# albertfgu/diffwave-sashimi

Hardware: AMD Instinct MI355X
Metric: audio samples/sec (generate.py-style reverse-diffusion sampling, T=200) (higher is better)
Workload: dtype f32-equivalent (3-term bf16 split, 6 products, fp32 accumulate); 1 GPU; wnet_h256_d36_T200; backbone=wavenet, batch_per_gpu=16, L=16000, T=200, parallelism=independent clips per GPU, no collective, sampler=hipGraph replay, on-device Philox noise

## Files before the change

### diffwave-sashimi_amd/csrc/bf16_split.h

```cpp
#pragma once
#include <hip/hip_runtime.h>

namespace dws {

typedef __bf16 bx_bf16x8 __attribute__((ext_vector_type(8)));
typedef __bf16 bx_bf16x4 __attribute__((ext_vector_type(4)));
typedef float bx_f32x16 __attribute__((ext_vector_type(16)));

__device__ __forceinline__ void split3(float x, __bf16& p0, __bf16& p1, __bf16& p2) {
    p0 = (__bf16)x;
    const float r1 = x - (float)p0;
    p1 = (__bf16)r1;
    const float r2 = r1 - (float)p1;
    p2 = (__bf16)r2;
}

__device__ __forceinline__ void split3x4(const float (&x)[4], bx_bf16x4& p0, bx_bf16x4& p1, bx_bf16x4& p2) {
#pragma unroll
    for (int e = 0; e < 4; ++e) {
        __bf16 a, b, c;
        split3(x[e], a, b, c);
        p0[e] = a; p1[e] = b; p2[e] = c;
    }
}
// ... 15 lines not shown
    out[1] = bx_bf16x8{a1, b1, z, z, z, z, z, z};
    out[2] = bx_bf16x8{a2, b2, z, z, z, z, z, z};
}

struct SplitBf16x3 {
    typedef bx_bf16x8 v8;
    typedef bx_bf16x4 v4;
    static constexpr int NT = 3, NP = 6;
    static constexpr bool SCALED = false;
    static constexpr float SX = 1.f, SG = 1.f;
    __device__ static constexpr int ia(int t) { return BX6_IA[t]; }
    __device__ static constexpr int ib(int t) { return BX6_IB[t]; }
    __device__ static __forceinline__ bx_f32x16 mfma(const v8& a, const v8& b, const bx_f32x16& c) {
        return __builtin_amdgcn_mfma_f32_32x32x16_bf16(a, b, c, 0, 0, 0);
    }
    __device__ static __forceinline__ void split4(const float (&x)[4], v4 (&p)[3]) { split3x4(x, p[0], p[1], p[2]); }
    __device__ static __forceinline__ void split1(float x, v8 (&out)[3], int i) {
        __bf16 a, b, c;
        split3(x, a, b, c);
        out[0][i] = a; out[1][i] = b; out[2][i] = c;
    }
    __device__ static __forceinline__ void rank2(float v0, float v1, bool lower_half, v8 (&out)[3]) { frag_rank2(v0, v1, lower_half, out); }
    __device__ static __forceinline__ void bits(float x, unsigned short (&b)[3]) {
        __bf16 p0, p1, p2;
        split3(x, p0, p1, p2);
        b[0] = __builtin_bit_cast(unsigned short, p0); b[1] = __builtin_bit_cast(unsigned short, p1); b[2] = __builtin_bit_cast(unsigned short, p2);
    }
    __device__ static __forceinline__ v8 bvals(float v0, float v1) {
        const __bf16 z = (__bf16)0.f;
        return v8{(__bf16)v0, (__bf16)v1, z, z, z, z, z, z};
    }
};

typedef _Float16 hx_f16x8 __attribute__((ext_vector_type(8)));
typedef _Float16 hx_f16x4 __attribute__((ext_vector_type(4)));
struct SplitF16x2 {
    typedef hx_f16x8 v8;
// ... 44 lines not shown
```

### diffwave-sashimi_amd/csrc/wavenet.h

```cpp
#pragma once
#include "dws_common.h"

namespace dws {

constexpr int WN_LAYER_KC = 32;
constexpr int WN_BX3_KC = 16;

struct WnLayerArgs {
    const float* x_in;
    float* x_out;
    float* skip;
    const float* part_t;
    int part_t_bstride;
    const float* A1;
    const float* A2;
    const float* Abt;
    int abt_bstride;
    const int* step_idx;
    int abt_tstride, part_t_tstride;
    const float* Wd;
    const float* Wr;
    const float* Ws;
    const float* bias1;
    const float* bias2;
// ... 36 lines not shown
bool wn_layer_mfma_supported(int C, int S);
int launch_wn_layer_mfma(int C, int S, const WnLayerArgs& a, hipStream_t s);
int launch_wn_layer_generic(int C, int S, const WnLayerArgs& a, hipStream_t s);
bool wn_final_mfma_supported(int S);
bool wn_layer_wino_supported(int C, int S);
int launch_wino_dconv(const float* w, float* out, int C, hipStream_t s);
int launch_wn_wino_bias(const float* Wd_all, const float* part_t, float* Abt, int NL, int B, int C, hipStream_t s);
int launch_wn_layer_wino(int C, int S, const WnLayerArgs& a, hipStream_t s);
bool wn_layer_bf16x3_supported(int C, int S);
int launch_wn_layer_bf16x3(int C, int S, const WnLayerArgs& a, hipStream_t s);
int launch_pack_a_bf16x3(const float* w, void* out, int M, int K, hipStream_t s);
int launch_wn_bias_tap_bf16(const float* Wd_all, const float* part_t, const float* bias1_all, void* Abt, int NL, int B, int C,
                            hipStream_t s);
enum { WN_SPLIT_BF16X6 = 0, WN_SPLIT_F16X3 = 1 };
inline int wn_split_terms(int split) { return split == WN_SPLIT_F16X3 ? 2 : 3; }
bool wn_layer_bx6_supported(int C, int S);
int launch_wn_layer_bx6(int C, int S, const WnLayerArgs& a, int split, hipStream_t s);
int launch_weight_scale(const float* w, size_t n, const float* bias, int nb, const float* bias_b, int nb_b, float* out, hipStream_t s);
int launch_pack_a1_bx6(const float* w, void* out, int C, int split, const float* scale, hipStream_t s);
int launch_pack_a_bx6(const float* w, void* out, int M, int K, int split, const float* scale, hipStream_t s);
int launch_gemm_bx6(const float* A, const float* B, float* C, int M, int N, int K, int split, float sa, float sb, hipStream_t s);
int launch_wn_final(int S, const WnFinalArgs& a, hipStream_t s);

}
```

### diffwave-sashimi_amd/csrc/wavenet_bx6.hip

```cpp
#include <cstdlib>
#include <type_traits>

#include "bf16_split.h"
#include "wavenet.h"
#include "wn_trace.h"

namespace dws {

#ifndef BX6_PF3
#define BX6_PF3 1
#endif
#ifndef BX6_PF2
#define BX6_PF2 2
#endif
#define BX6_PF(NT) ((NT) == 2 ? BX6_PF2 : BX6_PF3)
#ifndef BX6_T_SLOTS
#define BX6_T_SLOTS 0, 2, 3, 4, 6, 7, 9
#endif

typedef float bx6_f32x4 __attribute__((ext_vector_type(4)));

#ifdef BX6_ABL_NO_NT
#define BX6_NT 0
#else
// ... 120 lines not shown
    static constexpr int RAW_FLOATS = KC * 4 * NP;
    static constexpr int BOP_BYTES = (KC / 8) * 4 * NT * NP * 16;
    static constexpr int STAGE_FLOATS = 2 * RAW_FLOATS + 2 * BOP_BYTES / 4;
    static constexpr int GATE_BYTES = (C / 8) * NT * 64 * 16;
    static constexpr int MAIN_FLOATS = STAGE_FLOATS > GATE_BYTES / 4 ? STAGE_FLOATS : GATE_BYTES / 4;
    static constexpr int TR_FLOATS = 32 * 64;
    static constexpr int LDS_FLOATS = MAIN_FLOATS + WAVES * TR_FLOATS;
    static constexpr int TITEMS = (KC / 4) * NP * 2;
    static constexpr bool HALVES = WAVES == 8 && NT == 3;
    static constexpr int SW = HALVES ? WAVES / 2 : WAVES;
    static constexpr int NPIECE = KC / (2 * SW);
    static_assert(C % 32 == 0 && S % C == 0 && C % KC == 0 && KC % 16 == 0 && KC % (2 * SW) == 0 && (SW & (SW - 1)) == 0 &&
                  (!HALVES || NCB % 2 == 0) && (TITEMS % NTH == 0) && LDS_FLOATS * 4 <= 163840, "channel counts");
};

template <typename P, int C, int S, bool EXTRA>
__global__ __launch_bounds__(C * 2, (C >= 128 ? 2 : 1)) void wn_layer_bx6_kernel(WnLayerArgs a, int log2d) {
    using T = Bx6Tile<C, S, P::NT>;
    using v8 = typename P::v8;
    using v4 = typename P::v4;
    constexpr int NT = P::NT, NPR = P::NP, NA = 2 * P::NT;
    constexpr int KC = T::KC, MS = T::MS, WAVES = T::WAVES, NCB = T::NCB, NTH = T::NTH, NKB = T::NKB;
    __shared__ __attribute__((aligned(16))) float lds[T::LDS_FLOATS];
    float* const Xraw = lds;
    char* const Bop = reinterpret_cast<char*>(lds + 2 * T::RAW_FLOATS);
    char* const gt = reinterpret_cast<char*>(lds);

    const int tid = threadIdx.x;
    const int lane = tid & 63;
    const int wave = __builtin_amdgcn_readfirstlane(tid >> 6);
    const int l31 = lane & 31, lhi = lane >> 5;
    const int L = a.L, dil = 1 << log2d;
    float* const trw = lds + T::MAIN_FLOATS + wave * T::TR_FLOATS;
// ... 14 lines not shown
    const float* __restrict__ xb = a.x_in + (size_t)b * C * L;
    unsigned long long* __restrict__ trc = a.trace ? a.trace + ((size_t)blockIdx.x * WAVES + wave) * 32 : nullptr;
    auto stamp = [&](int i) {
        if (trc) {
            const unsigned long long t = __builtin_amdgcn_s_memtime();
            if (lane == 0) trc[i] = t;
        }
    };
    stamp(0);

    const int mt1[2] = {wave, C / 32 + wave};
    int mt2[1 + MS];
    mt2[0] = wave;
#pragma unroll
    for (int m = 0; m < MS; ++m) mt2[1 + m] = C / 32 + wave * MS + m;
    float av1[2][4], ab1[2], av2[1 + MS];
    {
        const float* Abt = a.Abt + (size_t)b * a.abt_bstride + step_row_off(a.step_idx, a.abt_tstride);
#pragma unroll
        for (int m = 0; m < 2; ++m) {
            const int row = mt1[m] * 32 + l31;
#pragma unroll
            for (int j = 0; j < 4; ++j) av1[m][j] = Abt[j * 2 * C + row];
            ab1[m] = a.bias1[row];
        }
#pragma unroll
        for (int m = 0; m < 1 + MS; ++m) av2[m] = a.bias2[mt2[m] * 32 + l31];
    }
    const float ws1 = P::SCALED ? a.wscale[0] : 1.f, ws2 = P::SCALED ? a.wscale[1] : 1.f;
    const float inv1 = 1.f / (ws1 * P::SX), inv2 = 1.f / (ws2 * P::SG);

    const bool al16 = (L % 4 == 0) && ((((size_t)a.x_in | (size_t)a.x_out | (size_t)a.skip) & 15) == 0);
// ... 132 lines not shown
#pragma unroll
        for (int m = 0; m < 2; ++m)
#pragma unroll
            for (int t = 0; t < NT; ++t)
#ifdef BX6_ABL_A_HOT
                dst[m][t] = __builtin_bit_cast(v8, __builtin_amdgcn_raw_buffer_load_b128(rA1, lane16, ((mt1[m] * NKB * 4) * NT + t) * 1024 + 0 * (kb + j), 0));
#else
                dst[m][t] = __builtin_bit_cast(v8, __builtin_amdgcn_raw_buffer_load_b128(rA1, lane16, (((mt1[m] * NKB + kb) * 4 + j) * NT + t) * 1024, 0));
#endif
    };

    if (stages(0)) stage_dma(0);
    if (NCB > 1 && stages(1)) stage_dma(1);
    constexpr int PF = BX6_PF(NT);
    v8 a_ring[4][2][NT];
#pragma unroll
    for (int s0 = 0; s0 < PF; ++s0) load_a1(a_ring[s0], chunk_of(0) * (KC / 16) + (s0 >> 2), s0 & 3);
    constexpr int NAF = PF * NA;
    constexpr int P16 = NPIECE + NAF, P4 = 4 * NPIECE + NAF;
    static_assert(P4 < 64, "vmcnt is a 6-bit counter");
    if (HALVES) {
        if (stages(0)) __builtin_amdgcn_s_waitcnt(0x0F70 | NAF);
    } else if (NCB > 1) {
        if (x4) __builtin_amdgcn_s_waitcnt(0x0F70 | (P16 & 15) | ((P16 >> 4) << 14));
        else __builtin_amdgcn_s_waitcnt(0x0F70 | (P4 & 15) | ((P4 >> 4) << 14));
    } else {
        __builtin_amdgcn_s_waitcnt(0x0F70 | NAF);
    }
    __syncthreads();
    stamp(1);
    {
        const float v0 = ((unsigned)(p - dil) < (unsigned)L) ? 1.f : 0.f;
        const float v1 = ((unsigned)p < (unsigned)L) ? 1.f : 0.f;
        const float v2 = ((unsigned)(p + dil) < (unsigned)L) ? 1.f : 0.f;
        const float v3 = ((unsigned)(p + 2 * dil) < (unsigned)L) ? 1.f : 0.f;
        const float bi[4] = {v0 - v2, v1 + v2, v2 - v1, v1 - v3};
        bx_f32x16 zero;
#pragma unroll
        for (int r = 0; r < 16; ++r) zero[r] = 0.f;
#pragma unroll
        for (int j = 0; j < 4; ++j) {
            const v8 bf = P::bvals(lhi ? 0.f : bi[j] * P::SX, (lhi || j != 1) ? 0.f : P::SX);
#pragma unroll
            for (int m = 0; m < 2; ++m) {
                v8 af[NT];
                P::rank2(av1[m][j] * ws1, j == 1 ? ab1[m] * ws1 : 0.f, lhi == 0, af);
// ... 60 lines not shown
        if constexpr (SPC == 4) {
            do_step(cb, std::integral_constant<int, 1>{}, std::false_type{});
            do_step(cb, std::integral_constant<int, 2>{}, std::false_type{});
            do_step(cb, std::integral_constant<int, 3>{}, std::false_type{});
        } else {
            do_step(cb, std::integral_constant<int, 1>{}, std::false_type{});
            do_step(cb, std::integral_constant<int, 2>{}, std::false_type{});
            do_step(cb, std::integral_constant<int, 3>{}, std::false_type{});
            do_step(cb, std::integral_constant<int, 4>{}, std::false_type{});
            do_step(cb, std::integral_constant<int, 5>{}, std::false_type{});
            do_step(cb, std::integral_constant<int, 6>{}, std::false_type{});
            do_step(cb, std::integral_constant<int, 7>{}, std::false_type{});
        }
    };
    static_assert((SPC == 4 || SPC == 8) && PF >= 1 && PF <= 3, "steps per chunk, prefetch distance");
    for (int cb = 0; cb < NCB; ++cb) {
#ifndef BX6_ABL_NO_STAGE
        if (cb + 2 < NCB && stages(cb + 2)) stage_dma(cb + 2);
#endif
        if (cb + 1 < NCB) do_step(cb, std::integral_constant<int, 0>{}, std::true_type{});
        else do_step(cb, std::integral_constant<int, 0>{}, std::false_type{});
        do_steps_from1(cb);
        stamp(8 + 2 * cb);
#ifndef BX6_ABL_NO_DMA_WAIT
        __builtin_amdgcn_s_waitcnt(0x0F70 | NAF);
#endif
#ifndef BX6_ABL_NO_BARRIER
        __syncthreads();
#endif
        stamp(9 + 2 * cb);
    }
    stamp(2);

    const int L4 = L * 4;
    const bool first = a.first_layer, last = a.last_layer;
    __amdgpu_buffer_rsrc_t rXo = __builtin_amdgcn_make_buffer_rsrc((void*)(a.x_out + (size_t)b * C * L), 0, C * L * 4, 0x00020000);
    __amdgpu_buffer_rsrc_t rSk = __builtin_amdgcn_make_buffer_rsrc((void*)(a.skip + (size_t)b * S * L), 0, S * L * 4, 0x00020000);
    const int p0 = ((q0 >> log2d) << (log2d + 1)) + (q0 & (dil - 1));
    int voff4;
    {
        const int n4 = (lane & 15) >> 3;
        const int pos4 = (contig ? pbase + 32 * n4 : p0 + n4 * dil) + 4 * (lane & 7);
        voff4 = (pos4 < L) ? ((lane >> 4) * L + pos4) * 4 : 0x7ffffff0;
    }
    constexpr bool PRELOAD = MS == 1;
    const int voff4s = first ? 0x7ffffff0 : voff4;
    auto load_pre = [&](int m, bx6_f32x4 (&dst)[8]) {
#pragma unroll
        for (int i = 0; i < 8; ++i) {
            if (m == 0) dst[i] = *reinterpret_cast<const bx6_f32x4*>(trw + ((lane >> 4) + 4 * i) * 64 + 4 * (lane & 15));
            else dst[i] = bx6_load_f4(rSk, voff4s, ((wave * MS + (m - 1)) * 32 + 4 * i) * L4);
        }
    };
    bx6_f32x4 pre[PRELOAD ? 1 + MS : 1][8];
    if (PRELOAD && al16) {
#pragma unroll
        for (int m = 1; m < 1 + MS; ++m) load_pre(m, pre[PRELOAD ? m : 0]);
    }

    const float* melb = (EXTRA && a.melc) ? a.melc + (size_t)(a.mel_bstride ? b : 0) * 2 * C * L : nullptr;
#pragma unroll
    for (int qd = 0; qd < 4; ++qd) {
        float g0[4], g1[4];
#pragma unroll
        for (int e = 0; e < 4; ++e) {
            const int r = qd * 4 + e;
            const int ch = wave * 32 + e + 8 * qd + 4 * lhi;
#pragma unroll
            for (int n = 0; n < 2; ++n) {
                const int pos = p + n * dil;
                float ht, hs;
                if (n == 0) {
                    ht = (acc[0][0][r] + acc[0][1][r]) + acc[0][2][r];
                    hs = (acc[1][0][r] + acc[1][1][r]) + acc[1][2][r];
                } else {
// ... 11 lines not shown
                    hb[(size_t)(C + ch) * L + pos] = hs;
                }
                const float g = bx6_gate(ht, hs) * P::SG;
                if (n == 0) g0[e] = g; else g1[e] = g;
            }
        }
        v4 s0[NT], s1[NT];
        P::split4(g0, s0);
        P::split4(g1, s1);
        char* dst = gt + ((wave * 4 + qd) * NT * 64) * 16 + lhi * 8;
#pragma unroll
        for (int t = 0; t < NT; ++t) {
            *reinterpret_cast<v4*>(dst + (t * 64 + gcol0) * 16) = s0[t];
            *reinterpret_cast<v4*>(dst + (t * 64 + gcol1) * 16) = s1[t];
        }
    }
    stamp(3);

    __amdgpu_buffer_rsrc_t rA2 = __builtin_amdgcn_make_buffer_rsrc((void*)a.A2, 0, (C + S) * C * 2 * NT, 0x00020000);
    v8 c_cur[1 + MS][NT], c_nxt[1 + MS][NT];
    auto load_a2 = [&](v8 (&dst)[1 + MS][NT], int kb, int m0) {
#pragma unroll
        for (int m = m0; m < 1 + MS; ++m)
#pragma unroll
            for (int t = 0; t < NT; ++t)
                dst[m][t] = __builtin_bit_cast(v8, __builtin_amdgcn_raw_buffer_load_b128(rA2, lane16, ((mt2[m] * NKB + kb) * NT + t) * 1024, 0));
    };
    const int rot2 = rot * (KC / 16);
    auto kblock_of = [&](int kb) { const int k = kb + rot2; return k >= NKB ? k - NKB : k; };
    bx_f32x16 acc2[1 + MS][2];
// ... 32 lines not shown
#pragma unroll
                for (int t = 0; t < NT; ++t) bq[n][t] = *reinterpret_cast<const v8*>(gk + (t * 64 + n * 32) * 16);
#pragma unroll
            for (int t = 0; t < NPR; ++t)
#pragma unroll
                for (int m = M0; m < 1 + MS; ++m)
#pragma unroll
                    for (int n = 0; n < 2; ++n)
                        acc2[m][n] = P::mfma(c_cur[m][P::ia(t)], bq[n][P::ib(t)], acc2[m][n]);
#pragma unroll
            for (int m = M0; m < 1 + MS; ++m)
#pragma unroll
                for (int t = 0; t < NT; ++t) c_cur[m][t] = c_nxt[m][t];
        }
    };
    if (last) gemm2(std::false_type{});
    else gemm2(std::true_type{});
    stamp(5);

    const float rs = 0.70710678118654752440f;
    if (al16) {
#pragma unroll
        for (int m = 0; m < 1 + MS; ++m) {
            if (m == 0 && last) continue;
            if (!PRELOAD || m == 0) load_pre(m, pre[0]);
            asm volatile("s_waitcnt lgkmcnt(0)" ::: "memory");
#pragma unroll
            for (int n = 0; n < 2; ++n)
#pragma unroll
                for (int r = 0; r < 16; ++r) trw[((r & 3) + 8 * (r >> 2) + 4 * lhi) * 64 + n * 32 + l31] = P::SCALED ? acc2[m][n][r] * inv2 : acc2[m][n][r];
            asm volatile("s_waitcnt lgkmcnt(0)" ::: "memory");
            const int row0 = (m == 0) ? wave * 32 : (wave * MS + (m - 1)) * 32;
#pragma unroll
            for (int i = 0; i < 8; ++i) {
                const bx6_f32x4 v = *reinterpret_cast<const bx6_f32x4*>(trw + ((lane >> 4) + 4 * i) * 64 + 4 * (lane & 15));
                bx6_f32x4 o = pre[PRELOAD ? m : 0][i] + v;
                if (m == 0) o = o * rs;
                bx6_store_f4(o, m == 0 ? rXo : rSk, voff4, (row0 + 4 * i) * L4);
                asm volatile("s_nop 1" ::: "memory");
            }
            asm volatile("" ::: "memory");
        }
    } else {
        int voffn[2];
#pragma unroll
        for (int n = 0; n < 2; ++n) {
            const int pos = contig ? pbase + 32 * n + l31 : p + n * dil;
            voffn[n] = (pos < L) ? (4 * lhi * L + pos) * 4 : 0x7ffffff0;
        }
#pragma unroll
        for (int n = 0; n < 2; ++n) {
            if (!last) {
                const int s0 = (wave * 32) * L4;
#pragma unroll
                for (int r = 0; r < 16; ++r) {
                    const int so = s0 + ((r & 3) + 8 * (r >> 2)) * L4;
                    const float x = __builtin_bit_cast(float, __builtin_amdgcn_raw_buffer_load_b32(rXall, voffn[n], so, 0));
// ... 9 lines not shown
                    const int so = s0 + ((r & 3) + 8 * (r >> 2)) * L4;
                    const float old = first ? 0.f : __builtin_bit_cast(float, __builtin_amdgcn_raw_buffer_load_b32(rSk, voffn[n], so, 0));
                    const float v = old + (P::SCALED ? acc2[1 + m][n][r] * inv2 : acc2[1 + m][n][r]);
                    __builtin_amdgcn_raw_buffer_store_b32(__builtin_bit_cast(unsigned, v), rSk, voffn[n], so, 0);
                }
            }
        }
    }
    stamp(6);
    if (trc) {
        __builtin_amdgcn_s_waitcnt(0);
        stamp(7);
    }
}

template <typename P, int C, int S>
static int launch_bx6_t(const WnLayerArgs& a, int log2d, hipStream_t s) {
    ProfileScope ps(P::NT == 3 ? "wn_layer_bx6" : "wn_layer_f16x3", s);
    using T = Bx6Tile<C, S, P::NT>;
    const int dil = 1 << log2d;
    const int nblk = (a.L + 2 * dil - 1) / (2 * dil);
    const int ntl = (nblk * dil + 31) / 32;
    const int ntiles = a.B * ntl;
    static const bool trace = std::getenv("DWS_BX6_TRACE") != nullptr;
    if (trace && !a.melc && !a.hsave) {
        wino_trace_launch(ntiles, T::WAVES, a, s, [&](const WnLayerArgs& at) {
            hipLaunchKernelGGL((wn_layer_bx6_kernel<P, C, S, false>), dim3(ntiles), dim3(T::NTH), 0, s, at, log2d);
        }, P::NT == 3 ? "bx6" : "f16x3");
        return DWS_OK;
    }
    if (a.melc || a.hsave) hipLaunchKernelGGL((wn_layer_bx6_kernel<P, C, S, true>), dim3(ntiles), dim3(T::NTH), 0, s, a, log2d);
    else hipLaunchKernelGGL((wn_layer_bx6_kernel<P, C, S, false>), dim3(ntiles), dim3(T::NTH), 0, s, a, log2d);
    return DWS_OK;
}

bool wn_layer_bx6_supported(int C, int S) {
    return (C == 64 && S == 64) || (C == 128 && S == 128) || (C == 128 && S == 256) || (C == 256 && S == 256);
}

template <typename P>
static int launch_bx6_p(int C, int S, const WnLayerArgs& a, int log2d, hipStream_t s) {
    if (C == 64 && S == 64) return launch_bx6_t<P, 64, 64>(a, log2d, s);
    if (C == 128 && S == 128) return launch_bx6_t<P, 128, 128>(a, log2d, s);
    if (C == 128 && S == 256) return launch_bx6_t<P, 128, 256>(a, log2d, s);
    if (C == 256 && S == 256) return launch_bx6_t<P, 256, 256>(a, log2d, s);
    return set_error(DWS_ERR_UNSUPPORTED, "wn_layer_bx6: (C=%d,S=%d) not instantiated", C, S);
}

int launch_wn_layer_bx6(int C, int S, const WnLayerArgs& a, int split, hipStream_t s) {
    int log2d = 0;
    while ((1 << log2d) < a.dilation) ++log2d;
    DWS_CHECK((1 << log2d) == a.dilation, DWS_ERR_UNSUPPORTED, "wn_layer_bx6: dilation %d is not a power of two", a.dilation);
    DWS_CHECK((int64_t)a.L + 4 * (int64_t)a.dilation < ((int64_t)1 << 28), DWS_ERR_UNSUPPORTED, "wn_layer_bx6: L too large");
    DWS_CHECK((int64_t)(C > S ? C : S) * a.L * 4 < ((int64_t)1 << 31), DWS_ERR_UNSUPPORTED,
              "wn_layer_bx6: %d channels x L=%d exceed a 2 GiB tensor per clip", C > S ? C : S, a.L);
    if (split == WN_SPLIT_F16X3) {
        DWS_CHECK(a.hsave == nullptr, DWS_ERR_UNSUPPORTED, "wn_layer_f16x3: the training forward runs with precision=f32 or bf16x6");
        DWS_CHECK(a.wscale != nullptr, DWS_ERR_INVALID, "wn_layer_f16x3: no weight scales");
        return launch_bx6_p<SplitF16x2>(C, S, a, log2d, s);
    }
    return launch_bx6_p<SplitBf16x3>(C, S, a, log2d, s);
}

template <typename P>
__global__ __launch_bounds__(64) void gemm_bx6_kernel(const float* __restrict__ A, const float* __restrict__ B, float* __restrict__ Cm,
                                                      int M, int N, int K, float sa, float sb) {
    using v8 = typename P::v8;
    const int lane = threadIdx.x, l31 = lane & 31, lhi = lane >> 5;
    const int mt = blockIdx.y, nt = blockIdx.x;
    bx_f32x16 acc;
#pragma unroll
    for (int r = 0; r < 16; ++r) acc[r] = 0.f;
    for (int kb = 0; kb < K / 16; ++kb) {
        v8 af[P::NT], bf[P::NT];
#pragma unroll
// ... 43 lines not shown
```

### diffwave-sashimi_amd/csrc/wavenet_model.hip

```cpp
#include <cmath>

#include "conditioner.h"
#include "model.h"
#include "wavenet.h"
#include "wavenet_backward.h"

namespace dws {

struct WaveNetModel : dws_model {
    int Cin, Cout, C, S, NL, cycle, Ein, Emid, Eout, MB;
    bool cond, mfma_layer, mfma_final;
    bool bf16x3 = false;
    bool bf16x6 = false;
    bool f16x3 = false;
    DevBuf wscale;
    bool wino_opt = true;
    bool wino_fits(int64_t nL) const {
        return (int64_t)std::max(C, S) * nL * 4 < ((int64_t)1 << 31) && nL + 4 * ((int64_t)1 << (cycle - 1)) < ((int64_t)1 << 28);
    }
    bool wino() const { return wino_opt && mfma_layer && !bf16x3 && !bf16x6 && !f16x3 && wn_layer_wino_supported(C, S) && (L == 0 || wino_fits(L)); }
    bool wino_rows() const { return wino() || bf16x6 || f16x3; }

    DevBuf Wi;
    std::vector<DevBuf> A1, Wrs, A2, bias2;
    DevBuf Wd_all;
    DevBuf Abt;
    DevBuf Wt_all, bt_all;
    DevBuf b1_all;
    DevBuf Wf, Af;
    DevBuf freq;
    CopyBatch stack_params, unstack_fc_t;
// ... 18 lines not shown
    DevBuf de_raw;
    bool trained_fwd = false;

    explicit WaveNetModel(const dws_model_desc& dd) {
        d = dd;
        Cin = d.in_channels; Cout = d.out_channels; C = d.res_channels; S = d.skip_channels;
        NL = d.num_res_layers; cycle = d.dilation_cycle;
        Ein = d.diffusion_step_embed_dim_in; Emid = d.diffusion_step_embed_dim_mid; Eout = d.diffusion_step_embed_dim_out;
        MB = d.mel_bands;
        cond = !d.unconditional;
        mfma_layer = wn_layer_mfma_supported(C, S);
        mfma_bwd = tapconv_mfma_supported(C, S, C, 1) && tapconv_mfma_supported(C, 2 * C, 0, 3) &&
                   tapconv_mfma_supported(S, S, 0, 1) && std::getenv("DWS_WAVENET_GENERIC_BWD") == nullptr;
        mfma_final = wn_final_mfma_supported(S);
        if (std::getenv("DWS_WN_DIRECT")) wino_opt = false;
        auto wn = [&](const std::string& p, std::vector<int64_t> vshape) {
            std::vector<int64_t> g(vshape.size(), 1);
            g[0] = vshape[0];
            add_param(p + ".bias", {vshape[0]});
            add_param(p + ".weight_g", g);
            add_param(p + ".weight_v", vshape);
        };
        wn("init_conv.0.conv", {C, Cin, 1});
        add_param("residual_layer.fc_t1.weight", {Emid, Ein});
        add_param("residual_layer.fc_t1.bias", {Emid});
        add_param("residual_layer.fc_t2.weight", {Eout, Emid});
        add_param("residual_layer.fc_t2.bias", {Eout});
        for (int n = 0; n < NL; ++n) {
            const std::string p = "residual_layer.residual_blocks." + std::to_string(n);
            add_param(p + ".fc_t.weight", {C, Eout});
// ... 34 lines not shown
                          "precision=bf16x6 is not built for (res_channels=%d, skip_channels=%d)", C, S);
                bf16x6 = true; bf16x3 = f16x3 = false; dirty = true; trained_fwd = false;
                return DWS_OK;
            }
            if (value == "f16x3") {
                DWS_CHECK(mfma_layer && wn_layer_bx6_supported(C, S), DWS_ERR_UNSUPPORTED,
                          "precision=f16x3 is not built for (res_channels=%d, skip_channels=%d)", C, S);
                f16x3 = true; bf16x3 = bf16x6 = false; dirty = true; trained_fwd = false;
                return DWS_OK;
            }
        }
        if (key == "conv_algo") {
            if (value == "winograd") { wino_opt = true; dirty = true; trained_fwd = false; return DWS_OK; }
            if (value == "direct") { wino_opt = false; dirty = true; trained_fwd = false; return DWS_OK; }
        }
        return dws_model::set_option(key, value);
    }

    float* Wd(int n) const { return Wd_all.f() + (size_t)n * 2 * C * C * 3; }

    int fold(const std::string& p, float* out, int O, int inner, hipStream_t s) {
        return launch_fold_weight_norm(P(p + ".weight_v"), P(p + ".weight_g"), out, O, inner, s);
    }

    int commit(hipStream_t s) override {
        DWS_TRY(Wi.ensure((size_t)C * Cin * 4));
        DWS_TRY(fold("init_conv.0.conv", Wi.f(), C, Cin, s));
        DWS_TRY(Wt_all.ensure((size_t)NL * C * Eout * 4));
        DWS_TRY(bt_all.ensure((size_t)NL * C * 4));
        DWS_TRY(b1_all.ensure((size_t)NL * 2 * C * 4));
        DWS_TRY(Wd_all.ensure((size_t)NL * 2 * C * C * 3 * 4));
        if (mfma_layer) DWS_TRY(tmp_pack.ensure((size_t)2 * C * 4 * C * 4));
        stack_params.begin();
        for (int n = 0; n < NL; ++n) {
            const std::string p = "residual_layer.residual_blocks." + std::to_string(n);
            stack_params.add(P(p + ".fc_t.weight"), Wt_all.f() + (size_t)n * C * Eout, (size_t)C * Eout);
            stack_params.add(P(p + ".fc_t.bias"), bt_all.f() + (size_t)n * C, (size_t)C);
            stack_params.add(P(p + ".dilated_conv_layer.conv.bias"), b1_all.f() + (size_t)n * 2 * C, (size_t)2 * C);
            DWS_TRY(fold(p + ".dilated_conv_layer.conv", Wd(n), 2 * C, C * 3, s));
            DWS_TRY(Wrs[n].ensure((size_t)(C + S) * C * 4));
// ... 321 lines not shown
                a.step_idx = step_idx;
            } else {
                a.part_t = part_t.f() + (size_t)n * C; a.part_t_bstride = NL * C;
                a.Abt = mfma_layer ? Abt.f() + (size_t)n * B * arow : nullptr; a.abt_bstride = arow;
            }
            a.Wd = Wd(n); a.Wr = Wrs[n].f(); a.Ws = Wrs[n].f() + (size_t)C * C;
            a.bias1 = P(p + ".dilated_conv_layer.conv.bias");
            a.bias2 = bias2[n].f();
            a.melc = melBm ? melc.f() + (size_t)n * melBm * 2 * C * L : nullptr;
            a.mel_bstride = (melBm > 1) ? 1 : 0;
            a.gate_ws = gate.f();
            a.B = (int)B; a.L = (int)L;
            a.dilation = 1 << (n % cycle);
            a.first_layer = (n == 0); a.last_layer = (n == NL - 1);
            if (mfma_layer && bf16x3) DWS_TRY(launch_wn_layer_bf16x3(C, S, a, s));
            else if (bf16x6) DWS_TRY(launch_wn_layer_bx6(C, S, a, WN_SPLIT_BF16X6, s));
            else if (f16x3) { a.wscale = wscale.f() + 2 * n; DWS_TRY(launch_wn_layer_bx6(C, S, a, WN_SPLIT_F16X3, s)); }
            else if (wino()) DWS_TRY(launch_wn_layer_wino(C, S, a, s));
            else if (mfma_layer) DWS_TRY(launch_wn_layer_mfma(C, S, a, s));
            else DWS_TRY(launch_wn_layer_generic(C, S, a, s));
        }
        DWS_TRY(final_stage(out, train ? ty.f() : nullptr, s));
        DWS_HIP(hipGetLastError());
        return DWS_OK;
    }

    int wn_bwd(const std::string& p, const float* dWf, int O, int inner, hipStream_t s) {
        return launch_weight_norm_bwd(dWf, P(p + ".weight_v"), P(p + ".weight_g"), G(p + ".weight_v"), G(p + ".weight_g"), O,
                                      inner, s);
    }

    int backward(const float* dout, float* daudio, bool pg, hipStream_t s) override {
// ... 191 lines not shown
```

Baseline: 33630 audio samples/s.

## Use 16x16x32 bf16 MFMA shape for both GEMMs in the bx6 WaveNet layer

Adds a variant of the bf16x6 WaveNet layer kernel for C=S=256 that issues 16x16x32 MFMAs instead of 32x32x16 for the dilated-conv GEMM, and optionally for the residual/skip GEMM. It restructures fragment loading, accumulator layout, the gate epilogue and the output stores to match, and becomes the default. The aim is better instruction scheduling, smaller accumulators and finer interleaving with the transform work. The cost is more complex indexing, per-element b32 stores in the epilogue, and higher register pressure.

```diff
diff --git a/diffwave-sashimi_amd/csrc/bf16_split.h b/diffwave-sashimi_amd/csrc/bf16_split.h
--- a/diffwave-sashimi_amd/csrc/bf16_split.h
+++ b/diffwave-sashimi_amd/csrc/bf16_split.h
@@ -6,6 +6,7 @@
 typedef __bf16 bx_bf16x8 __attribute__((ext_vector_type(8)));
 typedef __bf16 bx_bf16x4 __attribute__((ext_vector_type(4)));
 typedef float bx_f32x16 __attribute__((ext_vector_type(16)));
+typedef float bx_f32x4 __attribute__((ext_vector_type(4)));
 
 __device__ __forceinline__ void split3(float x, __bf16& p0, __bf16& p1, __bf16& p2) {
     p0 = (__bf16)x;
@@ -53,6 +54,9 @@
     __device__ static __forceinline__ bx_f32x16 mfma(const v8& a, const v8& b, const bx_f32x16& c) {
         return __builtin_amdgcn_mfma_f32_32x32x16_bf16(a, b, c, 0, 0, 0);
     }
+    __device__ static __forceinline__ bx_f32x4 mfma16(const v8& a, const v8& b, const bx_f32x4& c) {
+        return __builtin_amdgcn_mfma_f32_16x16x32_bf16(a, b, c, 0, 0, 0);
+    }
     __device__ static __forceinline__ void split4(const float (&x)[4], v4 (&p)[3]) { split3x4(x, p[0], p[1], p[2]); }
     __device__ static __forceinline__ void split1(float x, v8 (&out)[3], int i) {
         __bf16 a, b, c;
@@ -60,6 +64,11 @@
         out[0][i] = a; out[1][i] = b; out[2][i] = c;
     }
     __device__ static __forceinline__ void rank2(float v0, float v1, bool lower_half, v8 (&out)[3]) { frag_rank2(v0, v1, lower_half, out); }
+    __device__ static __forceinline__ void rank2_16(float v0, float v1, int lane, v8 (&out)[3]) { frag_rank2(v0, v1, (lane >> 4) == 0, out); }
+    __device__ static __forceinline__ v8 bvals_16(float v0, float v1, int lane) {
+        const bool k0 = (lane >> 4) == 0;
+        return bvals(k0 ? v0 : 0.f, k0 ? v1 : 0.f);
+    }
     __device__ static __forceinline__ void bits(float x, unsigned short (&b)[3]) {
         __bf16 p0, p1, p2;
         split3(x, p0, p1, p2);
diff --git a/diffwave-sashimi_amd/csrc/wavenet.h b/diffwave-sashimi_amd/csrc/wavenet.h
--- a/diffwave-sashimi_amd/csrc/wavenet.h
+++ b/diffwave-sashimi_amd/csrc/wavenet.h
@@ -74,8 +74,11 @@
                             hipStream_t s);
 enum { WN_SPLIT_BF16X6 = 0, WN_SPLIT_F16X3 = 1 };
 inline int wn_split_terms(int split) { return split == WN_SPLIT_F16X3 ? 2 : 3; }
+enum { WN_BX6_MFMA_32 = 0, WN_BX6_MFMA_G2_16 = 1, WN_BX6_MFMA_16 = 2 };
+constexpr int WN_BX6_MFMA_DEFAULT = WN_BX6_MFMA_16;
 bool wn_layer_bx6_supported(int C, int S);
-int launch_wn_layer_bx6(int C, int S, const WnLayerArgs& a, int split, hipStream_t s);
+bool wn_layer_bx6_mfma16_supported(int C, int S, int split);
+int launch_wn_layer_bx6(int C, int S, const WnLayerArgs& a, int split, int mfma, hipStream_t s);
 int launch_weight_scale(const float* w, size_t n, const float* bias, int nb, const float* bias_b, int nb_b, float* out, hipStream_t s);
 int launch_pack_a1_bx6(const float* w, void* out, int C, int split, const float* scale, hipStream_t s);
 int launch_pack_a_bx6(const float* w, void* out, int M, int K, int split, const float* scale, hipStream_t s);
diff --git a/diffwave-sashimi_amd/csrc/wavenet_bx6.hip b/diffwave-sashimi_amd/csrc/wavenet_bx6.hip
--- a/diffwave-sashimi_amd/csrc/wavenet_bx6.hip
+++ b/diffwave-sashimi_amd/csrc/wavenet_bx6.hip
@@ -158,9 +158,36 @@
                   (!HALVES || NCB % 2 == 0) && (TITEMS % NTH == 0) && LDS_FLOATS * 4 <= 163840, "channel counts");
 };
 
-template <typename P, int C, int S, bool EXTRA>
+enum { BX6_MF_32 = 0, BX6_MF_G2_16 = 1, BX6_MF_16 = 2 };
+#ifndef BX6_T16_SLOTS
+#define BX6_T16_SLOTS 1, 5, 7, 9, 13, 15, 19
+#endif
+struct Bx6Nothing {};
+template <int MS>
+struct Bx6G2State {
+    float bias[1 + MS][2];
+    bx_f32x4 acc[1 + MS][2][2][2];
+};
+template <int NT>
+__device__ __forceinline__ int bx6_voff_a1h(int lane) { return ((lane >> 5) * (4 * NT * 64) + ((lane >> 4) & 1) * 32 + (lane & 15)) * 16; }
+template <typename V8, int NT>
+__device__ __forceinline__ void bx6_load_a1h(V8 (&dst)[2][NT], __amdgpu_buffer_rsrc_t r, int voff, int soff) {
+#pragma unroll
+    for (int h = 0; h < 2; ++h)
+#pragma unroll
+        for (int t = 0; t < NT; ++t) dst[h][t] = __builtin_bit_cast(V8, __builtin_amdgcn_raw_buffer_load_b128(r, voff + h * 256, soff + t * 1024, 0));
+}
+template <typename V8, int NT>
+struct Bx6G1State {
+    float av[2][2][4], ab[2][2];
+    bx_f32x4 acc[2][4][2][2];
+    V8 ar[2][2][NT];
+    int pc[2];
+};
+template <typename P, int C, int S, bool EXTRA, int MF = BX6_MF_32>
 __global__ __launch_bounds__(C * 2, (C >= 128 ? 2 : 1)) void wn_layer_bx6_kernel(WnLayerArgs a, int log2d) {
     using T = Bx6Tile<C, S, P::NT>;
+    static_assert(MF == BX6_MF_32 || (P::NT == 3 && !P::SCALED && C == 256 && S == 256), "the 16x16x32 shape: bf16 split, C = S = 256");
     using v8 = typename P::v8;
     using v4 = typename P::v4;
     constexpr int NT = P::NT, NPR = P::NP, NA = 2 * P::NT;
@@ -205,8 +232,26 @@
     mt2[0] = wave;
 #pragma unroll
     for (int m = 0; m < MS; ++m) mt2[1 + m] = C / 32 + wave * MS + m;
+    [[maybe_unused]] std::conditional_t<MF >= BX6_MF_16, Bx6G1State<v8, NT>, Bx6Nothing> gs1;
+    if constexpr (MF >= BX6_MF_16) {
+        const float* Abt = a.Abt + (size_t)b * a.abt_bstride + step_row_off(a.step_idx, a.abt_tstride);
+#pragma unroll
+        for (int m = 0; m < 2; ++m)
+#pragma unroll
+            for (int h = 0; h < 2; ++h) {
+                const int row = (m ? C / 32 + wave : wave) * 32 + 16 * h + (lane & 15);
+#pragma unroll
+                for (int j = 0; j < 4; ++j) gs1.av[m][h][j] = Abt[j * 2 * C + row];
+                gs1.ab[m][h] = a.bias1[row];
+            }
+#pragma unroll
+        for (int c = 0; c < 2; ++c) {
+            const int qc = q0 + 16 * c + (lane & 15);
+            gs1.pc[c] = ((qc >> log2d) << (log2d + 1)) + (qc & (dil - 1));
+        }
+    }
     float av1[2][4], ab1[2], av2[1 + MS];
-    {
+    if constexpr (MF < BX6_MF_16) {
         const float* Abt = a.Abt + (size_t)b * a.abt_bstride + step_row_off(a.step_idx, a.abt_tstride);
 #pragma unroll
         for (int m = 0; m < 2; ++m) {
@@ -369,8 +414,13 @@
     if (NCB > 1 && stages(1)) stage_dma(1);
     constexpr int PF = BX6_PF(NT);
     v8 a_ring[4][2][NT];
+    if constexpr (MF >= BX6_MF_16) {
+        static_assert(MF < BX6_MF_16 || (PF == 1 && KC == 32), "one half-step of six fragments ahead: NAF and every vmcnt count as in the 32x32x16 form");
+        bx6_load_a1h<v8, NT>(gs1.ar[0], rA1, bx6_voff_a1h<NT>(lane), ((mt1[0] * NKB + 2 * chunk_of(0)) * 4 + 0) * NT * 1024);
+    } else {
 #pragma unroll
     for (int s0 = 0; s0 < PF; ++s0) load_a1(a_ring[s0], chunk_of(0) * (KC / 16) + (s0 >> 2), s0 & 3);
+    }
     constexpr int NAF = PF * NA;
     constexpr int P16 = NPIECE + NAF, P4 = 4 * NPIECE + NAF;
     static_assert(P4 < 64, "vmcnt is a 6-bit counter");
@@ -384,7 +434,35 @@
     }
     __syncthreads();
     stamp(1);
-    {
+    if constexpr (MF >= BX6_MF_16) {
+        const bx_f32x4 zero = {0.f, 0.f, 0.f, 0.f};
+        float bi[2][4];
+#pragma unroll
+        for (int c = 0; c < 2; ++c) {
+            const int pc = gs1.pc[c];
+            const float v0 = ((unsigned)(pc - dil) < (unsigned)L) ? 1.f : 0.f;
+            const float v1 = ((unsigned)pc < (unsigned)L) ? 1.f : 0.f;
+            const float v2 = ((unsigned)(pc + dil) < (unsigned)L) ? 1.f : 0.f;
+            const float v3 = ((unsigned)(pc + 2 * dil) < (unsigned)L) ? 1.f : 0.f;
+            bi[c][0] = v0 - v2; bi[c][1] = v1 + v2; bi[c][2] = v2 - v1; bi[c][3] = v1 - v3;
+        }
+#pragma unroll
+        for (int j = 0; j < 4; ++j)
+#pragma unroll
+            for (int m = 0; m < 2; ++m)
+#pragma unroll
+                for (int h = 0; h < 2; ++h) {
+                    v8 af[NT];
+                    P::rank2_16(gs1.av[m][h][j] * ws1, j == 1 ? gs1.ab[m][h] * ws1 : 0.f, lane, af);
+#pragma unroll
+                    for (int c = 0; c < 2; ++c) {
+                        const v8 bf = P::bvals_16(bi[c][j] * P::SX, j == 1 ? P::SX : 0.f, lane);
+                        gs1.acc[m][j][h][c] = zero;
+#pragma unroll
+                        for (int t = NT - 1; t >= 0; --t) gs1.acc[m][j][h][c] = P::mfma16(af[t], bf, gs1.acc[m][j][h][c]);
+                    }
+                }
+    } else {
         const float v0 = ((unsigned)(p - dil) < (unsigned)L) ? 1.f : 0.f;
         const float v1 = ((unsigned)p < (unsigned)L) ? 1.f : 0.f;
         const float v2 = ((unsigned)(p + dil) < (unsigned)L) ? 1.f : 0.f;
@@ -475,6 +553,69 @@
         }
     };
     static_assert((SPC == 4 || SPC == 8) && PF >= 1 && PF <= 3, "steps per chunk, prefetch distance");
+    if constexpr (MF >= BX6_MF_16) {
+        const int r16 = lane & 15, oct = lane >> 4;
+        const int voffa = bx6_voff_a1h<NT>(lane);
+        constexpr int T16_SLOTS[T_UNITS] = {BX6_T16_SLOTS};
+        v8 bq[2][NT], bq0[2][2];
+        auto do_half = [&](int cb, auto HS, auto WITH_T) {
+            constexpr int hs = decltype(HS)::value, j = hs >> 1, m = hs & 1;
+            constexpr bool ride = decltype(WITH_T)::value;
+            const char* tb = Bop + (cb & 1) * T::BOP_BYTES + oct * (4 * NT * 512) + r16 * 16;
+            if (hs == 2 && cb + 1 < NCB) keep_residual(cb + 1);
+            if (hs < 7) bx6_load_a1h<v8, NT>(gs1.ar[(hs + 1) & 1], rA1, voffa, ((mt1[(hs + 1) & 1] * NKB + 2 * chunk_of(cb)) * 4 + ((hs + 1) >> 1)) * NT * 1024);
+            else if (cb + 1 < NCB) bx6_load_a1h<v8, NT>(gs1.ar[0], rA1, voffa, ((mt1[0] * NKB + 2 * chunk_of(cb + 1)) * 4 + 0) * NT * 1024);
+            __builtin_amdgcn_sched_barrier(0);
+            if (hs == 0) {
+#pragma unroll
+                for (int t = 0; t < NT; ++t)
+#pragma unroll
+                    for (int c = 0; c < 2; ++c) (t ? bq[c][t] : bq0[0][c]) = *reinterpret_cast<const v8*>(tb + (j * NT + t) * 512 + c * 256);
+            }
+            if (m == 1 && j < 3) {
+#pragma unroll
+                for (int c = 0; c < 2; ++c) bq0[(j + 1) & 1][c] = *reinterpret_cast<const v8*>(tb + ((j + 1) * NT) * 512 + c * 256);
+            }
+            TState ts;
+#pragma unroll
+            for (int t = 0; t < NPR; ++t) {
+#pragma unroll
+                for (int h = 0; h < 2; ++h)
+#pragma unroll
+                    for (int c = 0; c < 2; ++c) {
+                        gs1.acc[m][j][h][c] = P::mfma16(gs1.ar[hs & 1][h][P::ia(t)], P::ib(t) ? bq[c][P::ib(t)] : bq0[j & 1][c], gs1.acc[m][j][h][c]);
+                        if (ride) {
+                            const int i = (2 * t + h) * 2 + c;
+#pragma unroll
+                            for (int u = 0; u < T_UNITS; ++u)
+                                if (T16_SLOTS[u] == i) transform_unit(cb + 1, u, ts);
+                            __builtin_amdgcn_sched_barrier(0);
+                        }
+                    }
+                if (m == 1 && j < 3 && (t == 2 || t == 4)) {
+                    const int term = (t == 2) ? 2 : 1;
+#pragma unroll
+                    for (int c = 0; c < 2; ++c) bq[c][term] = *reinterpret_cast<const v8*>(tb + ((j + 1) * NT + term) * 512 + c * 256);
+                }
+            }
+        };
+        for (int cb = 0; cb < NCB; ++cb) {
+            if (cb + 2 < NCB && stages(cb + 2)) stage_dma(cb + 2);
+            if (cb + 1 < NCB) do_half(cb, std::integral_constant<int, 0>{}, std::true_type{});
+            else do_half(cb, std::integral_constant<int, 0>{}, std::false_type{});
+            do_half(cb, std::integral_constant<int, 1>{}, std::false_type{});
+            do_half(cb, std::integral_constant<int, 2>{}, std::false_type{});
+            do_half(cb, std::integral_constant<int, 3>{}, std::false_type{});
+            do_half(cb, std::integral_constant<int, 4>{}, std::false_type{});
+            do_half(cb, std::integral_constant<int, 5>{}, std::false_type{});
+            do_half(cb, std::integral_constant<int, 6>{}, std::false_type{});
+            do_half(cb, std::integral_constant<int, 7>{}, std::false_type{});
+            stamp(8 + 2 * cb);
+            __builtin_amdgcn_s_waitcnt(0x0F70 | NAF);
+            __syncthreads();
+            stamp(9 + 2 * cb);
+        }
+    } else {
     for (int cb = 0; cb < NCB; ++cb) {
 #ifndef BX6_ABL_NO_STAGE
         if (cb + 2 < NCB && stages(cb + 2)) stage_dma(cb + 2);
@@ -491,8 +632,18 @@
 #endif
         stamp(9 + 2 * cb);
     }
+    }
     stamp(2);
-
+    int lane_t = lane;
+    if constexpr (MF >= BX6_MF_16) asm volatile("" : "+v"(lane_t));
+
+    [[maybe_unused]] std::conditional_t<MF >= BX6_MF_G2_16, Bx6G2State<MS>, Bx6Nothing> gs2;
+    if constexpr (MF >= BX6_MF_G2_16) {
+#pragma unroll
+        for (int m = 0; m < 1 + MS; ++m)
+#pragma unroll
+            for (int h = 0; h < 2; ++h) gs2.bias[m][h] = a.bias2[mt2[m] * 32 + 16 * h + (lane_t & 15)];
+    }
     const int L4 = L * 4;
     const bool first = a.first_layer, last = a.last_layer;
     __amdgpu_buffer_rsrc_t rXo = __builtin_amdgcn_make_buffer_rsrc((void*)(a.x_out + (size_t)b * C * L), 0, C * L * 4, 0x00020000);
@@ -500,16 +651,16 @@
     const int p0 = ((q0 >> log2d) << (log2d + 1)) + (q0 & (dil - 1));
     int voff4;
     {
-        const int n4 = (lane & 15) >> 3;
-        const int pos4 = (contig ? pbase + 32 * n4 : p0 + n4 * dil) + 4 * (lane & 7);
-        voff4 = (pos4 < L) ? ((lane >> 4) * L + pos4) * 4 : 0x7ffffff0;
+        const int n4 = (lane_t & 15) >> 3;
+        const int pos4 = (contig ? pbase + 32 * n4 : p0 + n4 * dil) + 4 * (lane_t & 7);
+        voff4 = (pos4 < L) ? ((lane_t >> 4) * L + pos4) * 4 : 0x7ffffff0;
     }
     constexpr bool PRELOAD = MS == 1;
     const int voff4s = first ? 0x7ffffff0 : voff4;
     auto load_pre = [&](int m, bx6_f32x4 (&dst)[8]) {
 #pragma unroll
         for (int i = 0; i < 8; ++i) {
-            if (m == 0) dst[i] = *reinterpret_cast<const bx6_f32x4*>(trw + ((lane >> 4) + 4 * i) * 64 + 4 * (lane & 15));
+            if (m == 0) dst[i] = *reinterpret_cast<const bx6_f32x4*>(trw + ((lane_t >> 4) + 4 * i) * 64 + 4 * (lane_t & 15));
             else dst[i] = bx6_load_f4(rSk, voff4s, ((wave * MS + (m - 1)) * 32 + 4 * i) * L4);
         }
     };
@@ -520,6 +671,55 @@
     }
 
     const float* melb = (EXTRA && a.melc) ? a.melc + (size_t)(a.mel_bstride ? b : 0) * 2 * C * L : nullptr;
+    if constexpr (MF >= BX6_MF_16) {
+        const int r16 = lane_t & 15, oct = lane_t >> 4;
+#pragma unroll
+        for (int c = 0; c < 2; ++c) {
+            const int qc = q0 + 16 * c + r16;
+            const int pc = ((qc >> log2d) << (log2d + 1)) + (qc & (dil - 1));
+            const int gc0 = contig ? pc - pbase : 16 * c + r16, gc1 = contig ? pc - pbase + dil : 32 + 16 * c + r16;
+#pragma unroll
+            for (int h = 0; h < 2; ++h) {
+                float ga[4], gb[4];
+#pragma unroll
+                for (int e = 0; e < 4; ++e) {
+                    const int ch = wave * 32 + 16 * h + 4 * oct + e;
+#pragma unroll
+                    for (int n = 0; n < 2; ++n) {
+                        const int pos = pc + n * dil;
+                        float ht, hs;
+                        if (n == 0) {
+                            ht = (gs1.acc[0][0][h][c][e] + gs1.acc[0][1][h][c][e]) + gs1.acc[0][2][h][c][e];
+                            hs = (gs1.acc[1][0][h][c][e] + gs1.acc[1][1][h][c][e]) + gs1.acc[1][2][h][c][e];
+                        } else {
+                            ht = (gs1.acc[0][1][h][c][e] - gs1.acc[0][2][h][c][e]) - gs1.acc[0][3][h][c][e];
+                            hs = (gs1.acc[1][1][h][c][e] - gs1.acc[1][2][h][c][e]) - gs1.acc[1][3][h][c][e];
+                        }
+                        if (EXTRA && melb && pos < L) {
+                            ht += melb[(size_t)ch * L + pos];
+                            hs += melb[(size_t)(C + ch) * L + pos];
+                        }
+                        if (EXTRA && a.hsave && pos < L) {
+                            float* __restrict__ hb = a.hsave + (size_t)b * 2 * C * L;
+                            hb[(size_t)ch * L + pos] = ht;
+                            hb[(size_t)(C + ch) * L + pos] = hs;
+                        }
+                        const float g = bx6_gate(ht, hs) * P::SG;
+                        if (n == 0) ga[e] = g; else gb[e] = g;
+                    }
+                }
+                v4 s0[NT], s1[NT];
+                P::split4(ga, s0);
+                P::split4(gb, s1);
+                char* dst = gt + ((wave * 4 + 2 * h + (oct >> 1)) * NT * 64) * 16 + (oct & 1) * 8;
+#pragma unroll
+                for (int t = 0; t < NT; ++t) {
+                    *reinterpret_cast<v4*>(dst + (t * 64 + gc0) * 16) = s0[t];
+                    *reinterpret_cast<v4*>(dst + (t * 64 + gc1) * 16) = s1[t];
+                }
+            }
+        }
+    } else {
 #pragma unroll
     for (int qd = 0; qd < 4; ++qd) {
         float g0[4], g1[4];
@@ -561,6 +761,7 @@
             *reinterpret_cast<v4*>(dst + (t * 64 + gcol0) * 16) = s0[t];
             *reinterpret_cast<v4*>(dst + (t * 64 + gcol1) * 16) = s1[t];
         }
+    }
     }
     stamp(3);
 
@@ -623,8 +824,80 @@
                 for (int t = 0; t < NT; ++t) c_cur[m][t] = c_nxt[m][t];
         }
     };
-    if (last) gemm2(std::false_type{});
-    else gemm2(std::true_type{});
+    if constexpr (MF >= BX6_MF_G2_16) {
+        auto gemm2_16 = [&](auto WITH_RES) {
+            const int r16 = lane_t & 15, oct = lane_t >> 4;
+            auto& acc2h = gs2.acc;
+            constexpr int M0 = decltype(WITH_RES)::value ? 0 : 1;
+            const int voffa = (oct >> 1) * (NT * 1024) + ((oct & 1) * 32 + r16) * 16;
+            auto load_a2h = [&](v8 (&dst)[1 + MS][NT], int kk, int h) {
+#pragma unroll
+                for (int m = M0; m < 1 + MS; ++m)
+#pragma unroll
+                    for (int t = 0; t < NT; ++t)
+                        dst[m][t] = __builtin_bit_cast(v8, __builtin_amdgcn_raw_buffer_load_b128(rA2, voffa + h * 256, ((mt2[m] * NKB + 2 * kk) * NT + t) * 1024, 0));
+            };
+            auto block_of = [&](int kk) { const int k = kk + rot; return k >= NCB ? k - NCB : k; };
+            static_assert(KC == 32, "GEMM2's rotation counts 32-channel blocks");
+            v8 ah[2][1 + MS][NT];
+            load_a2h(ah[0], block_of(0), 0);
+            {
+                const v8 bf = P::bvals_16(P::SG, 0.f, lane_t);
+                const bx_f32x4 zero = {0.f, 0.f, 0.f, 0.f};
+#pragma unroll
+                for (int m = M0; m < 1 + MS; ++m)
+#pragma unroll
+                    for (int h = 0; h < 2; ++h) {
+                        v8 af[NT];
+                        P::rank2_16(gs2.bias[m][h] * ws2, 0.f, lane_t, af);
+#pragma unroll
+                        for (int n = 0; n < 2; ++n)
+#pragma unroll
+                            for (int c = 0; c < 2; ++c) {
+                                acc2h[m][n][h][c] = zero;
+#pragma unroll
+                                for (int t = NT - 1; t >= 0; --t) acc2h[m][n][h][c] = P::mfma16(af[t], bf, acc2h[m][n][h][c]);
+                            }
+                    }
+            }
+            __syncthreads();
+            stamp(4);
+            const char* gb = gt + oct * (NT * 64 * 16) + r16 * 16;
+#pragma unroll 1
+            for (int kk = 0; kk < NCB; ++kk) {
+                const char* gk = gb + block_of(kk) * (4 * NT * 64 * 16);
+                v8 bq[2][2][NT];
+#pragma unroll
+                for (int h = 0; h < 2; ++h) {
+                    if (h == 0) load_a2h(ah[1], block_of(kk), 1);
+                    else load_a2h(ah[0], block_of(kk + 1 < NCB ? kk + 1 : kk), 0);
+                    __builtin_amdgcn_sched_barrier(0);
+                    if (h == 0) {
+#pragma unroll
+                        for (int n = 0; n < 2; ++n)
+#pragma unroll
+                            for (int c = 0; c < 2; ++c)
+#pragma unroll
+                                for (int t = 0; t < NT; ++t) bq[n][c][t] = *reinterpret_cast<const v8*>(gk + (t * 64 + n * 32 + c * 16) * 16);
+                    }
+#pragma unroll
+                    for (int t = 0; t < NPR; ++t)
+#pragma unroll
+                        for (int m = M0; m < 1 + MS; ++m)
+#pragma unroll
+                            for (int n = 0; n < 2; ++n)
+#pragma unroll
+                                for (int c = 0; c < 2; ++c)
+                                    acc2h[m][n][h][c] = P::mfma16(ah[h][m][P::ia(t)], bq[n][c][P::ib(t)], acc2h[m][n][h][c]);
+                }
+            }
+        };
+        if (last) gemm2_16(std::false_type{});
+        else gemm2_16(std::true_type{});
+    } else {
+        if (last) gemm2(std::false_type{});
+        else gemm2(std::true_type{});
+    }
     stamp(5);
 
     const float rs = 0.70710678118654752440f;
@@ -634,15 +907,29 @@
             if (m == 0 && last) continue;
             if (!PRELOAD || m == 0) load_pre(m, pre[0]);
             asm volatile("s_waitcnt lgkmcnt(0)" ::: "memory");
+            if constexpr (MF >= BX6_MF_G2_16) {
+                const int r16 = lane_t & 15, oct = lane_t >> 4;
+                auto& acc2h = gs2.acc;
+#pragma unroll
+                for (int n = 0; n < 2; ++n)
+#pragma unroll
+                    for (int h = 0; h < 2; ++h)
+#pragma unroll
+                        for (int c = 0; c < 2; ++c)
+#pragma unroll
+                            for (int r = 0; r < 4; ++r) trw[(16 * h + 4 * oct + r) * 64 + ((n * 32 + 16 * c + r16) ^ (oct << 4))] = acc2h[m][n][h][c][r];
+            } else {
 #pragma unroll
             for (int n = 0; n < 2; ++n)
 #pragma unroll
                 for (int r = 0; r < 16; ++r) trw[((r & 3) + 8 * (r >> 2) + 4 * lhi) * 64 + n * 32 + l31] = P::SCALED ? acc2[m][n][r] * inv2 : acc2[m][n][r];
+            }
             asm volatile("s_waitcnt lgkmcnt(0)" ::: "memory");
             const int row0 = (m == 0) ? wave * 32 : (wave * MS + (m - 1)) * 32;
 #pragma unroll
             for (int i = 0; i < 8; ++i) {
-                const bx6_f32x4 v = *reinterpret_cast<const bx6_f32x4*>(trw + ((lane >> 4) + 4 * i) * 64 + 4 * (lane & 15));
+                const bx6_f32x4 v = *reinterpret_cast<const bx6_f32x4*>(trw + ((lane_t >> 4) + 4 * i) * 64 +
+                                                                        (MF >= BX6_MF_G2_16 ? (4 * (lane_t & 15)) ^ ((i & 3) << 4) : 4 * (lane_t & 15)));
                 bx6_f32x4 o = pre[PRELOAD ? m : 0][i] + v;
                 if (m == 0) o = o * rs;
                 bx6_store_f4(o, m == 0 ? rXo : rSk, voff4, (row0 + 4 * i) * L4);
@@ -650,6 +937,40 @@
             }
             asm volatile("" ::: "memory");
         }
+    } else if constexpr (MF >= BX6_MF_G2_16) {
+        const int r16 = lane_t & 15, oct = lane_t >> 4;
+        auto& acc2h = gs2.acc;
+#pragma unroll
+        for (int n = 0; n < 2; ++n)
+#pragma unroll
+            for (int c = 0; c < 2; ++c) {
+                const int qc = q0 + 16 * c + r16;
+                const int pc = ((qc >> log2d) << (log2d + 1)) + (qc & (dil - 1));
+                const int pos = contig ? pbase + 32 * n + 16 * c + r16 : pc + n * dil;
+                const int voffc = (pos < L) ? (4 * oct * L + pos) * 4 : 0x7ffffff0;
+#pragma unroll
+                for (int h = 0; h < 2; ++h) {
+                    if (!last) {
+                        const int s0 = (wave * 32 + 16 * h) * L4;
+#pragma unroll
+                        for (int r = 0; r < 4; ++r) {
+                            const float x = __builtin_bit_cast(float, __builtin_amdgcn_raw_buffer_load_b32(rXall, voffc, s0 + r * L4, 0));
+                            const float v = (x + acc2h[0][n][h][c][r]) * rs;
+                            __builtin_amdgcn_raw_buffer_store_b32(__builtin_bit_cast(unsigned, v), rXo, voffc, s0 + r * L4, 0);
+                        }
+                    }
+#pragma unroll
+                    for (int m = 0; m < MS; ++m) {
+                        const int s0 = ((wave * MS + m) * 32 + 16 * h) * L4;
+#pragma unroll
+                        for (int r = 0; r < 4; ++r) {
+                            const float old = first ? 0.f : __builtin_bit_cast(float, __builtin_amdgcn_raw_buffer_load_b32(rSk, voffc, s0 + r * L4, 0));
+                            const float v = old + acc2h[1 + m][n][h][c][r];
+                            __builtin_amdgcn_raw_buffer_store_b32(__builtin_bit_cast(unsigned, v), rSk, voffc, s0 + r * L4, 0);
+                        }
+                    }
+                }
+            }
     } else {
         int voffn[2];
 #pragma unroll
@@ -689,7 +1010,7 @@
     }
 }
 
-template <typename P, int C, int S>
+template <typename P, int C, int S, int MF = BX6_MF_32>
 static int launch_bx6_t(const WnLayerArgs& a, int log2d, hipStream_t s) {
     ProfileScope ps(P::NT == 3 ? "wn_layer_bx6" : "wn_layer_f16x3", s);
     using T = Bx6Tile<C, S, P::NT>;
@@ -700,14 +1021,16 @@
     static const bool trace = std::getenv("DWS_BX6_TRACE") != nullptr;
     if (trace && !a.melc && !a.hsave) {
         wino_trace_launch(ntiles, T::WAVES, a, s, [&](const WnLayerArgs& at) {
-            hipLaunchKernelGGL((wn_layer_bx6_kernel<P, C, S, false>), dim3(ntiles), dim3(T::NTH), 0, s, at, log2d);
+            hipLaunchKernelGGL((wn_layer_bx6_kernel<P, C, S, false, MF>), dim3(ntiles), dim3(T::NTH), 0, s, at, log2d);
         }, P::NT == 3 ? "bx6" : "f16x3");
         return DWS_OK;
     }
-    if (a.melc || a.hsave) hipLaunchKernelGGL((wn_layer_bx6_kernel<P, C, S, true>), dim3(ntiles), dim3(T::NTH), 0, s, a, log2d);
-    else hipLaunchKernelGGL((wn_layer_bx6_kernel<P, C, S, false>), dim3(ntiles), dim3(T::NTH), 0, s, a, log2d);
+    if (a.melc || a.hsave) hipLaunchKernelGGL((wn_layer_bx6_kernel<P, C, S, true, MF>), dim3(ntiles), dim3(T::NTH), 0, s, a, log2d);
+    else hipLaunchKernelGGL((wn_layer_bx6_kernel<P, C, S, false, MF>), dim3(ntiles), dim3(T::NTH), 0, s, a, log2d);
     return DWS_OK;
 }
+
+bool wn_layer_bx6_mfma16_supported(int C, int S, int split) { return split == WN_SPLIT_BF16X6 && C == 256 && S == 256; }
 
 bool wn_layer_bx6_supported(int C, int S) {
     return (C == 64 && S == 64) || (C == 128 && S == 128) || (C == 128 && S == 256) || (C == 256 && S == 256);
@@ -722,7 +1045,7 @@
     return set_error(DWS_ERR_UNSUPPORTED, "wn_layer_bx6: (C=%d,S=%d) not instantiated", C, S);
 }
 
-int launch_wn_layer_bx6(int C, int S, const WnLayerArgs& a, int split, hipStream_t s) {
+int launch_wn_layer_bx6(int C, int S, const WnLayerArgs& a, int split, int mfma, hipStream_t s) {
     int log2d = 0;
     while ((1 << log2d) < a.dilation) ++log2d;
     DWS_CHECK((1 << log2d) == a.dilation, DWS_ERR_UNSUPPORTED, "wn_layer_bx6: dilation %d is not a power of two", a.dilation);
@@ -734,6 +1057,9 @@
         DWS_CHECK(a.wscale != nullptr, DWS_ERR_INVALID, "wn_layer_f16x3: no weight scales");
         return launch_bx6_p<SplitF16x2>(C, S, a, log2d, s);
     }
+    if (mfma == WN_BX6_MFMA_G2_16 && wn_layer_bx6_mfma16_supported(C, S, split)) return launch_bx6_t<SplitBf16x3, 256, 256, BX6_MF_G2_16>(a, log2d, s);
+    if (mfma == WN_BX6_MFMA_16 && wn_layer_bx6_mfma16_supported(C, S, split)) return launch_bx6_t<SplitBf16x3, 256, 256, BX6_MF_16>(a, log2d, s);
+    DWS_CHECK(mfma == WN_BX6_MFMA_32 || mfma == WN_BX6_MFMA_G2_16 || mfma == WN_BX6_MFMA_16, DWS_ERR_INVALID, "wn_layer_bx6: unknown MFMA shape %d", mfma);
     return launch_bx6_p<SplitBf16x3>(C, S, a, log2d, s);
 }
 
diff --git a/diffwave-sashimi_amd/csrc/wavenet_model.hip b/diffwave-sashimi_amd/csrc/wavenet_model.hip
--- a/diffwave-sashimi_amd/csrc/wavenet_model.hip
+++ b/diffwave-sashimi_amd/csrc/wavenet_model.hip
@@ -15,6 +15,14 @@
     bool f16x3 = false;
     DevBuf wscale;
     bool wino_opt = true;
+    int bx6_mfma = WN_BX6_MFMA_DEFAULT;
+    bool bx6_mfma_env_bad = false;
+    static bool parse_bx6_mfma(const std::string& v, int& out) {
+        if (v == "32x32x16") { out = WN_BX6_MFMA_32; return true; }
+        if (v == "gemm2-16x16x32") { out = WN_BX6_MFMA_G2_16; return true; }
+        if (v == "16x16x32") { out = WN_BX6_MFMA_16; return true; }
+        return false;
+    }
     bool wino_fits(int64_t nL) const {
         return (int64_t)std::max(C, S) * nL * 4 < ((int64_t)1 << 31) && nL + 4 * ((int64_t)1 << (cycle - 1)) < ((int64_t)1 << 28);
     }
@@ -63,6 +71,7 @@
                    tapconv_mfma_supported(S, S, 0, 1) && std::getenv("DWS_WAVENET_GENERIC_BWD") == nullptr;
         mfma_final = wn_final_mfma_supported(S);
         if (std::getenv("DWS_WN_DIRECT")) wino_opt = false;
+        if (const char* e = std::getenv("DWS_BX6_MFMA")) bx6_mfma_env_bad = !parse_bx6_mfma(e, bx6_mfma);
         auto wn = [&](const std::string& p, std::vector<int64_t> vshape) {
             std::vector<int64_t> g(vshape.size(), 1);
             g[0] = vshape[0];
@@ -127,6 +136,12 @@
             if (value == "winograd") { wino_opt = true; dirty = true; trained_fwd = false; return DWS_OK; }
             if (value == "direct") { wino_opt = false; dirty = true; trained_fwd = false; return DWS_OK; }
         }
+        if (key == "bx6_mfma") {
+            int v = 0;
+            DWS_CHECK(parse_bx6_mfma(value, v), DWS_ERR_INVALID, "bx6_mfma: 32x32x16 | gemm2-16x16x32 | 16x16x32, not '%s'", value.c_str());
+            bx6_mfma = v; bx6_mfma_env_bad = false; dirty = true; trained_fwd = false;
+            return DWS_OK;
+        }
         return dws_model::set_option(key, value);
     }
 
@@ -137,6 +152,7 @@
     }
 
     int commit(hipStream_t s) override {
+        DWS_CHECK(!bx6_mfma_env_bad, DWS_ERR_INVALID, "DWS_BX6_MFMA: 32x32x16 | gemm2-16x16x32 | 16x16x32, not '%s'", std::getenv("DWS_BX6_MFMA") ? std::getenv("DWS_BX6_MFMA") : "");
         DWS_TRY(Wi.ensure((size_t)C * Cin * 4));
         DWS_TRY(fold("init_conv.0.conv", Wi.f(), C, Cin, s));
         DWS_TRY(Wt_all.ensure((size_t)NL * C * Eout * 4));
@@ -488,8 +504,8 @@
             a.dilation = 1 << (n % cycle);
             a.first_layer = (n == 0); a.last_layer = (n == NL - 1);
             if (mfma_layer && bf16x3) DWS_TRY(launch_wn_layer_bf16x3(C, S, a, s));
-            else if (bf16x6) DWS_TRY(launch_wn_layer_bx6(C, S, a, WN_SPLIT_BF16X6, s));
-            else if (f16x3) { a.wscale = wscale.f() + 2 * n; DWS_TRY(launch_wn_layer_bx6(C, S, a, WN_SPLIT_F16X3, s)); }
+            else if (bf16x6) DWS_TRY(launch_wn_layer_bx6(C, S, a, WN_SPLIT_BF16X6, bx6_mfma, s));
+            else if (f16x3) { a.wscale = wscale.f() + 2 * n; DWS_TRY(launch_wn_layer_bx6(C, S, a, WN_SPLIT_F16X3, WN_BX6_MFMA_32, s)); }
             else if (wino()) DWS_TRY(launch_wn_layer_wino(C, S, a, s));
             else if (mfma_layer) DWS_TRY(launch_wn_layer_mfma(C, S, a, s));
             else DWS_TRY(launch_wn_layer_generic(C, S, a, s));
```

New measurement: 34230 audio samples/s, median of 6. 1.02x the previous value.
